# rojas-diego/tokengeex

Measured on AMD Instinct MI355X. Metric: MB/s raw bytes encoded (and tokens/s) at 32K/64K vocab, 1/2/4/8 GPUs, higher is better.
Workload: dtype f64

## Files before the change

### tokengeex_amd/csrc/encode2.hip

```cpp
#include <hip/hip_runtime.h>
#include <stdint.h>

#include "device_common.h"
#include "kernels.h"
#include "trace_body.h"

namespace tgx {

constexpr uint32_t kNoStep2 = 0xFFu;
constexpr uint32_t kRows2Bytes = 64u * 32u * 8u;
constexpr uint64_t kHiHalf = 0xFFFFFFFF00000000ULL;

template <int U>
__device__ __forceinline__ void relax2_step(double sv, double& acc, uint32_t& bpv, uint32_t& fin, uint32_t& fhi) {
    constexpr uint64_t MU = (1ULL << U) | (1ULL << (32 + U));
    fin = sel_u32(MU, bpv, fin);
    fhi = sel_u32(MU, (uint32_t)((uint64_t)__double_as_longlong(acc) >> 32), fhi);
    const double b0 = readlane_f64(acc, (uint32_t)U), b1 = readlane_f64(acc, 32u + (uint32_t)U);
    const double best = sel_f64(kHiHalf, b1, b0);
    const double cand = best + sv;
    const uint64_t take = __builtin_amdgcn_fcmp(cand, acc, 2 ) | MU;
    acc = sel_f64(take, cand, acc);
    bpv = sel_imm_u32<U>(take, bpv);
}
// ... 74 lines not shown
            if (alive) {
                const uint32_t c = (bytes[d >> 2] >> ((d & 3) * 8)) & 0xFFu;
                const uint32_t t = base ^ c;
                const uint4 rec = load_rec(trie, t);
                alive = rec.x == cur;
                if (alive) {
                    cur = t;
                    base = rec.y & 0x7FFFFFFFu;
                    bool term = (rec.y >> 31) != 0u;
                    if (DROPOUT) {
                        if (term && d >= 1) term = P.dropout < dropout_u01(P.seed, s, pg, (uint32_t)d + 1u);
                    }
                    if (term) scw[((uint32_t)d + l) & 31u] = __hiloint2double((int)rec.w, (int)rec.z);
                }
            }
        }
        __builtin_amdgcn_wave_barrier();
        {
            const uint32_t* __restrict__ np = wp + 8;
#pragma unroll
            for (int q = 0; q < 9; ++q) wn[q] = np[q];
        }

        uint32_t fin = kNoStep2, fhi = 0xFFF00000u;
        {
            const double* scr = sc + r * 1024u + ((l - 1u) & 31u);
            double sv[16];
#pragma unroll
            for (int u = 0; u < 16; ++u) sv[u] = scr[u * 32];
            relax2_step<0>(sv[0], acc, bpv, fin, fhi);
            relax2_step<1>(sv[1], acc, bpv, fin, fhi);
            relax2_step<2>(sv[2], acc, bpv, fin, fhi);
            relax2_step<3>(sv[3], acc, bpv, fin, fhi);
            relax2_step<4>(sv[4], acc, bpv, fin, fhi);
            relax2_step<5>(sv[5], acc, bpv, fin, fhi);
            relax2_step<6>(sv[6], acc, bpv, fin, fhi);
            relax2_step<7>(sv[7], acc, bpv, fin, fhi);
            relax2_step<8>(sv[8], acc, bpv, fin, fhi);
            relax2_step<9>(sv[9], acc, bpv, fin, fhi);
            relax2_step<10>(sv[10], acc, bpv, fin, fhi);
            relax2_step<11>(sv[11], acc, bpv, fin, fhi);
            relax2_step<12>(sv[12], acc, bpv, fin, fhi);
            relax2_step<13>(sv[13], acc, bpv, fin, fhi);
            relax2_step<14>(sv[14], acc, bpv, fin, fhi);
            relax2_step<15>(sv[15], acc, bpv, fin, fhi);
#pragma unroll
            for (int u = 0; u < 16; ++u) sv[u] = scr[(u + 16) * 32];
            relax2_step<16>(sv[0], acc, bpv, fin, fhi);
            relax2_step<17>(sv[1], acc, bpv, fin, fhi);
            relax2_step<18>(sv[2], acc, bpv, fin, fhi);
            relax2_step<19>(sv[3], acc, bpv, fin, fhi);
            relax2_step<20>(sv[4], acc, bpv, fin, fhi);
            relax2_step<21>(sv[5], acc, bpv, fin, fhi);
            relax2_step<22>(sv[6], acc, bpv, fin, fhi);
            relax2_step<23>(sv[7], acc, bpv, fin, fhi);
            relax2_step<24>(sv[8], acc, bpv, fin, fhi);
            relax2_step<25>(sv[9], acc, bpv, fin, fhi);
            relax2_step<26>(sv[10], acc, bpv, fin, fhi);
            relax2_step<27>(sv[11], acc, bpv, fin, fhi);
            relax2_step<28>(sv[12], acc, bpv, fin, fhi);
            relax2_step<29>(sv[13], acc, bpv, fin, fhi);
            relax2_step<30>(sv[14], acc, bpv, fin, fhi);
            relax2_step<31>(sv[15], acc, bpv, fin, fhi);
        }
        __builtin_amdgcn_wave_barrier();
        const bool reached = fhi != 0xFFF00000u;

        if (live && pg >= 1u && pg <= n) {
            const uint8_t b = reached ? (uint8_t)((l - fin - 1u) & 31u) : (uint8_t)0xFF;
            __builtin_nontemporal_store(b, P.bp8 + bp8_base(beg, s) + (PERM ? bp8_perm(pg - 1u) : pg - 1u));
        }
        if (live) {
            const uint32_t left = n - p0;
            if (left < 32u) {
                if (left == l) P.status[s] = (n == 0u || reached) ? 1u : 0u;
                need_new = true;
            } else {
                p0 += 32u;
            }
        }
    }
}

template <bool PERM, bool CARRY>
__global__ __launch_bounds__(256) void trace32_kernel(EncodeParams P) {
    __shared__ typename TraceRingEntry<CARRY>::type ring_all[4][kTraceRing];
    trace_body<32, PERM, false, CARRY>(P, ring_all[threadIdx.x >> 6]);
}

hipError_t launch_encode2(const EncodeParams& p, uint32_t num_cus, bool permuted, hipStream_t stream) {
    const uint32_t waves = 5, bpc = 2;
    const uint64_t want = (p.n_samples + 2 * waves - 1) / (2 * waves);
    const uint32_t blocks = (uint32_t)(want < (uint64_t)num_cus * bpc ? (want ? want : 1) : (uint64_t)num_cus * bpc);
    auto fn = p.dropout > 0.0 ? (permuted ? encode2_kernel<true, true> : encode2_kernel<true, false>)
                              : (permuted ? encode2_kernel<false, true> : encode2_kernel<false, false>);
    hipError_t e = hipFuncSetAttribute(reinterpret_cast<const void*>(fn), hipFuncAttributeMaxDynamicSharedMemorySize, 160 * 1024);
    if (e != hipSuccess) return e;
    hipLaunchKernelGGL(fn, dim3(blocks), dim3(64u * waves), waves * kRows2Bytes, stream, p);
    return hipGetLastError();
}
hipError_t launch_trace32(const EncodeParams& p, uint32_t blocks, bool permuted, hipStream_t stream) {
    auto fn = permuted ? (p.trace_carry ? trace32_kernel<true, true> : trace32_kernel<true, false>)
                       : (p.trace_carry ? trace32_kernel<false, true> : trace32_kernel<false, false>);
    hipLaunchKernelGGL(fn, dim3(blocks), dim3(256), 0, stream, p);
    return hipGetLastError();
}

}
```

### tokengeex_amd/csrc/kernels.h

```cpp
#pragma once
#include <hip/hip_runtime.h>
#include <stdint.h>

#include "decode.h"
#include "spans.h"

namespace tgx {

struct EncodeParams {
    const uint8_t* text;
    const uint64_t* offs;
    const uint32_t* order;
    uint64_t n_samples;
    const void* trie;
    const uint32_t* tokid;
    uint32_t root_base;
    uint32_t n_slots;
    uint32_t lm;
    uint32_t* bp;
    uint32_t* tmp;
    uint32_t* counts;
    uint32_t* status;
    uint8_t* bp8;
    const void* tokhash;
    uint32_t tokhash_mask;
    uint32_t tokhash_seed;
    unsigned long long* err_sample;
    unsigned long long* queue;
    unsigned long long* redo_count;
    uint32_t* redo_list;
    double dropout;
    uint64_t seed;
    uint32_t flags;
    unsigned long long* stamps;
    uint32_t trace_carry;
};

struct Encode5Params {
    const void* trie8;
    uint32_t trie_bytes;
    const double* values;
    uint32_t root_base;
    uint32_t n_values;
    uint32_t n_hot;
    uint32_t claim_chunk;
    uint32_t list_off, root_off, idx_off;
    uint32_t ctrl_off, ring_off, ring_slots;
    uint32_t pool;
    unsigned int* started;
};

struct CompactParams {
    const uint64_t* offs;
    const uint32_t* order;
    uint64_t n_samples;
    const uint32_t* tmp;
    const uint64_t* out_offs;
    uint32_t* ids;
};

struct EstepParams {
    const uint8_t* text;
    const uint64_t* offs;
    const uint32_t* order;
    uint64_t n_samples;
    const void* trie_fwd;
    const void* trie_rev;
    uint32_t root_fwd, root_rev;
    uint32_t lm;
    uint64_t snippet_len;
    double* alpha;
    double* expected_slot;
    uint32_t n_slots_rev, n_replicas;
    double* logz_sum;
    unsigned long long* err_sample;
    double dropout;
    uint64_t seed;
};

hipError_t launch_pair_keys(const uint32_t* ids, const uint64_t* out_offs, uint64_t n_samples, uint32_t shift,
                            unsigned long long sentinel, unsigned long long* keys, uint32_t blocks, hipStream_t stream);
hipError_t pair_sort_temp_bytes(uint64_t n, size_t* bytes);
hipError_t pair_sort(void* temp, size_t temp_bytes, const unsigned long long* in, unsigned long long* out,
                     uint64_t n, unsigned int end_bit, hipStream_t stream);
hipError_t pair_rle_temp_bytes(uint64_t n, size_t* bytes);
hipError_t pair_rle(void* temp, size_t temp_bytes, const unsigned long long* sorted, uint64_t n,
                    unsigned long long* unique_out, unsigned int* counts_out, unsigned int* n_runs_out,
                    hipStream_t stream);

hipError_t pair_count_sort_temp_bytes(uint64_t n, size_t* bytes);
hipError_t pair_count_sort(void* temp, size_t temp_bytes, const unsigned int* counts_in, unsigned int* counts_out,
                           const unsigned long long* keys_in, unsigned long long* keys_out, uint64_t n,
                           hipStream_t stream);
hipError_t launch_pair_expand(const unsigned long long* keys, const unsigned int* cnt, uint64_t n, uint32_t shift,
                              unsigned long long* out_keys, unsigned long long* out_counts, hipStream_t stream);
constexpr uint32_t kHistMaxVocab = 36864;
hipError_t launch_ids_histogram(const uint32_t* ids, uint64_t n, uint32_t vocab, unsigned long long* out, uint32_t blocks,
                                hipStream_t stream);
hipError_t ids_sort_temp_bytes(uint64_t n, size_t* bytes);
hipError_t ids_sort(void* temp, size_t temp_bytes, const uint32_t* in, uint32_t* out, uint64_t n,
                    unsigned int end_bit, hipStream_t stream);
hipError_t ids_rle_temp_bytes(uint64_t n, size_t* bytes);
hipError_t ids_rle(void* temp, size_t temp_bytes, const uint32_t* sorted, uint64_t n, uint32_t* unique_out,
                   unsigned int* counts_out, unsigned int* n_runs_out, hipStream_t stream);

struct Estep4Params {
    const uint8_t* text;
    const uint64_t* soffs;
    const uint32_t* order;
    uint64_t n_snips;
    const uint32_t* snip_sample;
    const uint64_t* snip_base;
    const void* trie_fwd;
    const void* trie_rev;
    uint32_t root_fwd, root_rev;
    double* alpha;
    double* zarr;
    int32_t* alpha_exp;
// ... 241 lines not shown
```

### tokengeex_amd/csrc/kernels.hip

```cpp
#include <hip/hip_runtime.h>
#include <stdint.h>

#include <rocprim/device/device_scan.hpp>
#include <rocprim/iterator/transform_iterator.hpp>

#include "kernels.h"
#include "trace_body.h"
#include "device_common.h"

namespace tgx {

struct WaveCtx {
    const uint4* __restrict__ trie;
    uint32_t root_base;
    double dropout;
    uint64_t seed;
    bool use_dropout;
    uint32_t flags;
};

__device__ __forceinline__ void block_generic(const WaveCtx& C, const uint8_t* __restrict__ text, uint32_t n,
                                              uint32_t s, uint32_t p0, uint32_t lane, uint32_t LM,
                                              double* sc, uint32_t* hl, uint8_t* txt, uint32_t* __restrict__ bp,
                                              double& acc, uint32_t& bpv, uint64_t& reach, uint32_t& reach_n) {
// ... 394 lines not shown
                    }
                }
            }
        }
        __builtin_amdgcn_wave_barrier();
        TGX_STAMP(2)
        {
            const uint32_t* __restrict__ np = wp + 4 * PPL;
#pragma unroll
            for (int q = 0; q <= 4 * PPL; ++q) wn[q] = np[q];
        }

        uint32_t fin[PPL];
        bool reached[PPL];
#pragma unroll
        for (int g = 0; g < PPL; ++g) {
            fin[g] = kNoStep;
            reached[g] = false;
            if (P.flags & 2u) continue;
            const double* scr = reinterpret_cast<const double*>(wbase + g * kRows4GroupBytes) + r * 256u + ((l - 1u) & 15u);
            double sv[16];
#pragma unroll
            for (int u = 0; u < 16; ++u) sv[u] = scr[u * 16];
            uint32_t fhi = 0xFFF00000u;
            relax5_step<0>(sv[0], acc, bpv, fin[g], fhi);
            relax5_step<1>(sv[1], acc, bpv, fin[g], fhi);
            relax5_step<2>(sv[2], acc, bpv, fin[g], fhi);
            relax5_step<3>(sv[3], acc, bpv, fin[g], fhi);
            relax5_step<4>(sv[4], acc, bpv, fin[g], fhi);
            relax5_step<5>(sv[5], acc, bpv, fin[g], fhi);
            relax5_step<6>(sv[6], acc, bpv, fin[g], fhi);
            relax5_step<7>(sv[7], acc, bpv, fin[g], fhi);
            relax5_step<8>(sv[8], acc, bpv, fin[g], fhi);
            relax5_step<9>(sv[9], acc, bpv, fin[g], fhi);
            relax5_step<10>(sv[10], acc, bpv, fin[g], fhi);
            relax5_step<11>(sv[11], acc, bpv, fin[g], fhi);
            relax5_step<12>(sv[12], acc, bpv, fin[g], fhi);
            relax5_step<13>(sv[13], acc, bpv, fin[g], fhi);
            relax5_step<14>(sv[14], acc, bpv, fin[g], fhi);
            relax5_step<15>(sv[15], acc, bpv, fin[g], fhi);
            reached[g] = fhi != 0xFFF00000u;
        }
        __builtin_amdgcn_wave_barrier();
        TGX_STAMP(3)

        uint8_t* const bpw = P.bp8 + bp8_base(beg, s);
#pragma unroll
        for (int g = 0; g < PPL; ++g)
            if (live && pg[g] >= 1u && pg[g] <= n) {
                const uint32_t b = reached[g] ? ((l - fin[g] - 1u) & 15u) : 0xFFu;
                const uint32_t j = pg[g] - 1u, kq = (j >> 4) & 3u;
                pk = (kq == 0u) ? b : (pk | (b << (8u * kq)));
                pk_j = j;
                pk_dirty = true;
                if (kq == 3u) {
                    __builtin_nontemporal_store(pk, reinterpret_cast<uint32_t*>(bpw + (bp8_perm(j) & ~3u)));
                    pk_dirty = false;
                }
            }
        if (live && n - p0 < SPAN && pk_dirty) {
            __builtin_nontemporal_store(pk, reinterpret_cast<uint32_t*>(bpw + (bp8_perm(pk_j) & ~3u)));
            pk_dirty = false;
        }
        if (live) {
            const uint32_t left = n - p0;
            if (left < SPAN) {
#pragma unroll
                for (int g = 0; g < PPL; ++g)
                    if (left == 16u * g + l) P.status[s] = (n == 0u || reached[g]) ? 1u : 0u;
                need_new = true;
            } else {
                p0 += SPAN;
            }
        }
        TGX_STAMP(4)
    }
    if (STAMP && lane == 0 && P.stamps) {
        unsigned long long* o = P.stamps + (size_t)(blockIdx.x * wpb + wave) * 8u;
        for (int i = 0; i < 5; ++i) o[i] = seg[i];
        o[5] = iters;
    }
}

template <bool STAMP, bool CARRY>
__global__ __launch_bounds__(256) void trace_kernel(EncodeParams P) {
    __shared__ typename TraceRingEntry<CARRY>::type ring_all[4][kTraceRing];
    trace_body<16, true, STAMP, CARRY>(P, ring_all[threadIdx.x >> 6]);
}

__global__ __launch_bounds__(1024) void scan_counts_kernel(const uint32_t* __restrict__ counts,
                                                           uint64_t* __restrict__ offsets,
                                                           uint64_t n) {
    __shared__ uint64_t wsum[16];
    __shared__ uint64_t carry_s;
    constexpr uint32_t E = 8;
    const uint32_t tid = threadIdx.x, lane = tid & 63u, wave = tid >> 6;
    if (tid == 0) carry_s = 0;
    __syncthreads();
    for (uint64_t base = 0; base < n; base += 1024u * E) {
        const uint64_t i0 = base + (uint64_t)tid * E;
        uint32_t c[E];
        uint64_t v = 0;
#pragma unroll
        for (uint32_t e = 0; e < E; ++e) {
            c[e] = (i0 + e < n) ? counts[i0 + e] : 0u;
            v += c[e];
        }
        uint64_t x = v;
        for (int off = 1; off < 64; off <<= 1) {
            uint64_t y = __shfl_up(x, off);
            if ((int)lane >= off) x += y;
        }
        if (lane == 63) wsum[wave] = x;
        __syncthreads();
        uint64_t wprefix = 0;
        for (uint32_t w = 0; w < wave; ++w) wprefix += wsum[w];
        const uint64_t carry = carry_s;
        uint64_t run = carry + wprefix + x - v;
#pragma unroll
        for (uint32_t e = 0; e < E; ++e) {
            if (i0 + e < n) offsets[i0 + e] = run;
            run += c[e];
        }
        __syncthreads();
        if (tid == 1023) carry_s = run;
        __syncthreads();
    }
    if (tid == 0) offsets[n] = carry_s;
}

template <bool ROWS>
__global__ __launch_bounds__(256) void compact_kernel(CompactParams P) {
    const uint32_t lane = threadIdx.x & 63u;
    const uint32_t sub = ROWS ? (lane & 15u) : lane, width = ROWS ? 16u : 64u;
    const uint64_t n_units = (uint64_t)gridDim.x * 4u * (ROWS ? 4u : 1u);
    const uint32_t wave_id = blockIdx.x * 4u + (threadIdx.x >> 6);
    for (uint64_t k = ROWS ? (uint64_t)wave_id * 4u + (lane >> 4) : (uint64_t)wave_id; k < P.n_samples; k += n_units) {
        const uint32_t s = ROWS ? (uint32_t)k : P.order[k];
        const uint64_t end = P.offs[s + 1];
        const uint64_t o0 = P.out_offs[s];
        const uint32_t cnt = (uint32_t)(P.out_offs[s + 1] - o0);
        const uint32_t* __restrict__ src = P.tmp + (end - cnt);
        uint32_t* __restrict__ dst = P.ids + o0;
        struct __attribute__((packed, aligned(4))) Ids4 { uint32_t w[4]; };
        const uint32_t body = cnt & ~3u;
        for (uint32_t i = sub * 4u; i < body; i += width * 4u)
            *reinterpret_cast<Ids4*>(dst + i) = *reinterpret_cast<const Ids4*>(src + i);
        if (body + sub < cnt) dst[body + sub] = src[body + sub];
    }
}


static int lmt_for(uint32_t lm) { return lm <= 16u ? 16 : (lm <= 32u ? 32 : 0); }
uint32_t encode_effective_lm(uint32_t lm) {
    const int t = lmt_for(lm);
    return t ? (uint32_t)t : lm;
}

uint32_t encode_waves_per_block(uint32_t lm) {
    uint32_t w = (64u * 1024u) / wave_lds_bytes(encode_effective_lm(lm));
    return w < 1u ? 1u : (w > 4u ? 4u : w);
}
uint32_t encode_lds_bytes_per_block(uint32_t lm) {
    return encode_waves_per_block(lm) * wave_lds_bytes(encode_effective_lm(lm));
}

typedef void (*encode_fn)(EncodeParams);
static encode_fn pick_kernel(uint32_t lm) {
    const int t = lmt_for(lm);
    if (t == 16) return encode_kernel<16>;
    if (t == 32) return encode_kernel<32>;
    return encode_kernel<0>;
}

hipError_t launch_encode(const EncodeParams& p, uint32_t blocks, hipStream_t stream) {
    const uint32_t lds = encode_lds_bytes_per_block(p.lm);
    const dim3 block(64u * encode_waves_per_block(p.lm));
    hipLaunchKernelGGL(pick_kernel(p.lm), dim3(blocks), block, lds, stream, p);
    return hipGetLastError();
}

hipError_t encode_max_blocks_per_cu(uint32_t lm, int* out) {
    const uint32_t lds = encode_lds_bytes_per_block(lm);
    const int threads = (int)(64u * encode_waves_per_block(lm));
    if (lds > 160u * 1024u) return hipErrorInvalidValue;
    encode_fn fn = pick_kernel(lm);
    hipError_t e = hipFuncSetAttribute(reinterpret_cast<const void*>(fn),
                                       hipFuncAttributeMaxDynamicSharedMemorySize, (int)lds);
    if (e != hipSuccess) return e;
    return hipOccupancyMaxActiveBlocksPerMultiprocessor(out, fn, threads, lds);
}

typedef void (*encode4_fn)(EncodeParams);
static encode4_fn pick_encode4(bool dropout, int ppl, bool stamp, bool root) {
    if (stamp) return encode4_kernel<false, 1, true, false>;
    if (root) return dropout ? encode4_kernel<true, 1, false, true> : encode4_kernel<false, 1, false, true>;
    if (ppl == 1) return dropout ? encode4_kernel<true, 1, false, false> : encode4_kernel<false, 1, false, false>;
    if (ppl == 2) return dropout ? encode4_kernel<true, 2, false, false> : encode4_kernel<false, 2, false, false>;
    return dropout ? encode4_kernel<true, 4, false, false> : encode4_kernel<false, 4, false, false>;
}
uint32_t encode4_group_bytes() { return kRows4GroupBytes; }
uint32_t encode4_lds_bytes(int waves, int ppl, bool root) {
    return (root ? 4096u : 0u) + (uint32_t)waves * (uint32_t)ppl * kRows4GroupBytes;
}
hipError_t encode4_waves_per_simd(bool dropout, int ppl, bool root, int* out) {
    root = root && ppl == 1;
    hipFuncAttributes attr;
    hipError_t e = hipFuncGetAttributes(&attr, reinterpret_cast<const void*>(pick_encode4(dropout, ppl, false, root)));
    if (e != hipSuccess) return e;
    const int regs = (attr.numRegs + 7) & ~7;
    *out = regs > 0 ? (512 / regs > 8 ? 8 : 512 / regs) : 8;
    return hipSuccess;
}
hipError_t launch_encode4(const EncodeParams& p, int ppl, int waves, uint32_t blocks, bool root, hipStream_t stream) {
    const bool stamp = p.stamps != nullptr;
    root = root && !stamp && ppl == 1;
    encode4_fn fn = pick_encode4(p.dropout > 0.0, ppl, stamp, root);
    hipError_t e = hipFuncSetAttribute(reinterpret_cast<const void*>(fn), hipFuncAttributeMaxDynamicSharedMemorySize, 160 * 1024);
    if (e != hipSuccess) return e;
    hipLaunchKernelGGL(fn, dim3(blocks), dim3(64u * (uint32_t)waves), encode4_lds_bytes(waves, stamp ? 1 : ppl, root), stream, p);
    return hipGetLastError();
}
hipError_t launch_trace(const EncodeParams& p, uint32_t blocks, hipStream_t stream) {
    if (p.stamps)
        hipLaunchKernelGGL((trace_kernel<true, false>), dim3(blocks), dim3(256), 0, stream, p);
    else if (p.trace_carry)
        hipLaunchKernelGGL((trace_kernel<false, true>), dim3(blocks), dim3(256), 0, stream, p);
    else
        hipLaunchKernelGGL((trace_kernel<false, false>), dim3(blocks), dim3(256), 0, stream, p);
    return hipGetLastError();
}

struct WidenU32 {
    __host__ __device__ uint64_t operator()(uint32_t x) const { return (uint64_t)x; }
};
hipError_t scan_temp_bytes(uint64_t n, size_t* bytes) {
    *bytes = 0;
    if (n <= 65536) return hipSuccess;
    auto in = rocprim::make_transform_iterator((const uint32_t*)nullptr, WidenU32());
    return rocprim::exclusive_scan(nullptr, *bytes, in, (uint64_t*)nullptr, (uint64_t)0, (size_t)(n + 1), rocprim::plus<uint64_t>());
}
hipError_t launch_scan(uint32_t* counts, uint64_t* offsets, uint64_t n, void* temp, size_t temp_bytes, hipStream_t stream) {
    if (n <= 65536 || !temp) {
        hipLaunchKernelGGL(scan_counts_kernel, dim3(1), dim3(1024), 0, stream, counts, offsets, n);
        return hipGetLastError();
    }
    hipError_t e = hipMemsetAsync(counts + n, 0, 4, stream);
    if (e != hipSuccess) return e;
    auto in = rocprim::make_transform_iterator((const uint32_t*)counts, WidenU32());
    return rocprim::exclusive_scan(temp, temp_bytes, in, offsets, (uint64_t)0, (size_t)(n + 1), rocprim::plus<uint64_t>(), stream);
}

hipError_t launch_compact(const CompactParams& p, uint32_t blocks, bool rows, hipStream_t stream) {
    if (rows)
        hipLaunchKernelGGL(compact_kernel<true>, dim3(blocks), dim3(256), 0, stream, p);
    else
        hipLaunchKernelGGL(compact_kernel<false>, dim3(blocks), dim3(256), 0, stream, p);
    return hipGetLastError();
}

}
```

### tokengeex_amd/csrc/tgx_api.cpp

```cpp
#include <hip/hip_runtime.h>

#include <algorithm>
#include <unordered_set>
#include <cstdarg>
#include <cstddef>
#include <cstdio>
#include <cstdlib>
#include <cmath>
#include <cstring>
#include <chrono>
#include <condition_variable>
#include <memory>
#include <mutex>
#include <new>
#include <numeric>
#include <string>
#include <thread>
#include <vector>

#include "../../include/tgx.h"
#include "api_internal.h"
#include "assemble.h"
#include "decode.h"
#include "kernels.h"
// ... 473 lines not shown

tgx_status ensure_value_ranks(tgx_model* m, const tgx_corpus* c) {
    if (m->values_ranked || !m->have_trie8 || !c->n_bytes) return TGX_OK;
    m->values_ranked = true;
    const char* vr = knob("TGX_VALUE_RANK");
    if (vr && strcmp(vr, "model") == 0) return TGX_OK;
    if (m->n_values <= tgx::encode5_max_hot(false, 13, 3, 160u * 1024u) && !(vr && strcmp(vr, "counts") == 0)) return TGX_OK;
    tgx::HostPhases hp("ensure_value_ranks");
    HIP_TRY(hipSetDevice(m->device));
    const uint32_t nv = m->n_values, chunk = 65536u;
    const uint64_t stride = std::max<uint64_t>(chunk, (c->n_bytes + 63) / 64);
    const size_t cb = ((size_t)nv + 1) * 4 + 256;
    Pass pass(m);
    unsigned int* d_cnt = nullptr;
    uint32_t* d_perm = nullptr;
    if (pass.alloc(cb, &d_cnt) != hipSuccess || pass.alloc(cb, &d_perm) != hipSuccess)
        return fail(TGX_ERR_DEVICE, "out of device memory (value counts)");
    std::vector<unsigned int> cnt((size_t)nv + 1, 0u);
    std::vector<double> values((size_t)nv + 1), wvalues;
    bool ok = hipMemsetAsync(d_cnt, 0, cb, m->stream) == hipSuccess &&
              tgx::launch_value_count(c->d_text, c->n_bytes, chunk, stride, m->d_trie8, (uint32_t)m->flat.table.size(), m->root_base8, nv,
                                      std::max<uint32_t>(1, m->flat.max_token_len), d_cnt, (uint32_t)m->num_cus, m->stream) == hipSuccess &&
              hipMemcpyAsync(cnt.data(), d_cnt, ((size_t)nv + 1) * 4, hipMemcpyDeviceToHost, m->stream) == hipSuccess &&
              hipMemcpyAsync(values.data(), m->d_values, ((size_t)nv + 1) * 8, hipMemcpyDeviceToHost, m->stream) == hipSuccess;
    if (ok && m->have_wvalues) {
        wvalues.resize((size_t)nv + 1);
        ok = hipMemcpyAsync(wvalues.data(), m->d_wvalues, ((size_t)nv + 1) * 8, hipMemcpyDeviceToHost, m->stream) == hipSuccess;
    }
    if (!ok || hipStreamSynchronize(m->stream) != hipSuccess)
        return fail(TGX_ERR_DEVICE, "value count pass failed: %s", hipGetErrorString(hipGetLastError()));
    hp.mark("value counts");
    std::vector<uint32_t> order(nv);
    for (uint32_t r = 0; r < nv; r++) order[r] = r + 1u;
    std::stable_sort(order.begin(), order.end(), [&](uint32_t a, uint32_t b) { return cnt[a] > cnt[b]; });
    std::vector<uint32_t> perm((size_t)nv + 1, 0u);
    std::vector<double> v2((size_t)nv + 1), w2(wvalues.size());
    v2[0] = values[0];
    if (!w2.empty()) w2[0] = wvalues[0];
    unsigned long long total = 0, run = 0;
    for (uint32_t r = 0; r < nv; r++) total += cnt[order[r]];
    std::vector<double> cov((size_t)nv + 1, 0.0);
    for (uint32_t r = 0; r < nv; r++) {
        perm[order[r]] = r + 1u;
        v2[r + 1u] = values[order[r]];
        if (!w2.empty()) w2[r + 1u] = wvalues[order[r]];
        run += cnt[order[r]];
        cov[r + 1u] = total ? (double)run / (double)total : 1.0;
    }
    cov[nv] = 1.0;
    ok = hipMemcpyAsync(d_perm, perm.data(), ((size_t)nv + 1) * 4, hipMemcpyHostToDevice, m->stream) == hipSuccess &&
         tgx::launch_rank_remap(m->d_trie8, (uint32_t)m->flat.table.size(), d_perm, m->stream) == hipSuccess &&
         hipMemcpyAsync(m->d_values, v2.data(), ((size_t)nv + 1) * 8, hipMemcpyHostToDevice, m->stream) == hipSuccess &&
         (w2.empty() || hipMemcpyAsync(m->d_wvalues, w2.data(), ((size_t)nv + 1) * 8, hipMemcpyHostToDevice, m->stream) == hipSuccess) &&
         hipStreamSynchronize(m->stream) == hipSuccess;
    if (!ok) return fail(TGX_ERR_DEVICE, "value re-rank failed: %s", hipGetErrorString(hipGetLastError()));
    m->value_coverage = std::move(cov);
    hp.mark("re-rank");
    return pass.done();
}

tgx::EncodeParams base_encode_params(const tgx_model* m, const tgx_corpus* c, uint64_t seed) {
    tgx::EncodeParams p{};
    p.text = c->d_text;
    p.offs = c->d_offs;
    p.order = c->d_order;
    p.n_samples = c->n_samples;
    p.trie = m->d_trie;
    p.tokid = m->d_tokid;
    p.root_base = m->flat.table[0].base & ~tgx::kTerminalBit;
    p.lm = m->lm;
    p.n_slots = (uint32_t)m->flat.table.size();
    p.bp = c->d_bp;
    p.tmp = c->d_tmp;
    p.counts = c->d_counts;
    p.status = c->d_status;
    p.bp8 = reinterpret_cast<uint8_t*>(c->d_bp.get());
    p.tokhash = m->d_tokhash;
    p.tokhash_mask = m->tokhash.mask;
    p.tokhash_seed = m->tokhash.seed;
    p.err_sample = &m->d_ctrl->err;
    p.queue = &m->d_ctrl->queue;
    p.seed = seed;
    p.trace_carry = (c->n_samples && c->n_bytes / c->n_samples < 2048) ? 1u : 0u;
    return p;
}

tgx_status redo_long_matches(tgx_model* m, tgx_corpus* c, const tgx::EncodeParams& p) {
    unsigned long long n_redo = 0;
    HIP_TRY(hipMemcpyAsync(&n_redo, &m->d_ctrl->encode_redo, 8, hipMemcpyDeviceToHost, m->stream));
    HIP_TRY(hipStreamSynchronize(m->stream));
    if (n_redo > c->n_samples) return fail(TGX_ERR_DEVICE, "redo list longer than the batch");
    m->last_redo_samples = n_redo;
    if (n_redo) {
        tgx::EncodeParams q = p;
        q.order = c->d_counts;
        q.n_samples = n_redo;
        HIP_TRY(hipMemsetAsync(&m->d_ctrl->queue, 0x00, 8, m->stream));
        time_begin(m, "encode2_kernel");
        HIP_TRY(tgx::launch_encode2(q, (uint32_t)m->num_cus, true, m->stream));
        time_end(m);
    }
    return TGX_OK;
}

tgx_status run_encode_kernel(tgx_model* m, tgx_corpus* c, double dropout, uint64_t seed, Pass& pass) {
    tgx_status st = ensure_scratch(c);
    if (st != TGX_OK) return st;
    HIP_TRY(hipMemsetAsync(&m->d_ctrl->queue, 0x00, 8, m->stream));
    HIP_TRY(hipMemsetAsync(&m->d_ctrl->err, 0xFF, 8, m->stream));
    tgx::EncodeParams p = base_encode_params(m, c, seed);
    p.dropout = dropout;
    if (const char* e = knob("TGX_TRACE_CARRY")) p.trace_carry = atoi(e) ? 1u : 0u;
    p.flags = debug_flags();
    const char* force = knob("TGX_PATH");
    const bool use4 = m->lm <= 16 && m->scores_finite && m->d_tokhash && !(force && strcmp(force, "fused") == 0);
    const bool use2 = !use4 && m->lm <= 32 && m->scores_finite && m->d_tokhash && !(force && strcmp(force, "fused") == 0);
    const bool long_tokens = m->lm > 16;
    const bool use5 = (use4 || use2) && m->have_trie8 &&
                      !(force && (strcmp(force, "rows4") == 0 || strcmp(force, "rows2") == 0 || strcmp(force, "rows4l") == 0));
    if (debug_on())
        fprintf(stderr, "[tgx] encode: S=%llu N=%llu lm=%u path=%s slots=%zu root_base=%u values=%u\n",
                (unsigned long long)c->n_samples, (unsigned long long)c->n_bytes, p.lm, use4 ? (use5 ? "rows5" : "rows4") : (use2 ? "rows2" : "fused"),
                m->flat.table.size(), p.root_base, m->n_values);
    if (use5) {
        {
            const tgx_status rst = ensure_value_ranks(m, c);
            if (rst != TGX_OK) return rst;
        }
        m->last_redo_samples = 0;
        int e6_bpc = 2;
        if (const char* e = knob("TGX_E6_BPC")) e6_bpc = std::min(4, std::max(1, atoi(e)));
        uint32_t n_hot6 = std::min(m->n_values, tgx::encode6_max_hot(160u * 1024u / (uint32_t)e6_bpc, 0u));
        uint32_t pool6 = 0;
        bool e6_usable = true;
        if (n_hot6 < m->n_values) {
            pool6 = 128;
            if (const char* e = knob("TGX_E6_POOL")) pool6 = (uint32_t)std::min(192, std::max(0, atoi(e)));
            if ((uint64_t)m->n_values + tgx::encode6_pool_total(pool6) > 65535ull) {
                pool6 = 0;
                e6_usable = knob("TGX_E6_POOL") != nullptr || knob("TGX_LONG_THRESHOLD") != nullptr;
            }
            n_hot6 = std::min(m->n_values, tgx::encode6_max_hot(160u * 1024u / (uint32_t)e6_bpc, pool6));
        }
        n_hot6 = knob_cap_hot("TGX_E5_HOT", n_hot6);
        const bool cold6 = n_hot6 < m->n_values;
        uint64_t n_long = 0;
        uint32_t corun_cus = 0;
        if (c->n_samples && !long_tokens && e6_usable) {
            const auto count_ge = [&](uint64_t thr) {
                return (uint64_t)(std::partition_point(c->h_sorted_len.begin(), c->h_sorted_len.end(),
                                                       [thr](uint32_t len) { return len >= thr; }) - c->h_sorted_len.begin());
            };
            if (const char* e = knob("TGX_LONG_THRESHOLD")) {
                const uint64_t thr = (uint64_t)std::max(0ll, atoll(e));
                if (thr) n_long = count_ge(thr);
            } else {
                const double N = (double)c->n_bytes;
                const double c5 = m->n_values > tgx::encode5_max_hot(false, 8, 4, 160u * 1024u) ? 0.135e-6 : 0.108e-6;
                auto cost = [&](uint64_t k) {
                    const double bytes_long = k ? (double)c->h_sorted_cum[k - 1] : 0.0;
                    const double t6 = k ? std::max((double)c->h_sorted_len[0] * (cold6 ? 0.042e-6 : 0.0369e-6), bytes_long / (cold6 ? 46e9 : 55e9)) + 20e-6 : 0.0;
                    const double rest_max = k < c->n_samples ? (double)c->h_sorted_len[k] : 0.0;
                    const double t5 = std::max(rest_max * c5, (N - bytes_long) / 88e9);
                    return t6 + t5;
                };
                double best = cost(0);
                for (uint64_t thr = 1024; thr <= c->max_len; thr *= 2) {
                    const uint64_t k = count_ge(thr);
                    const double ck = cost(k);
                    if (k && ck < best * 0.9) {
                        best = ck;
                        n_long = k;
                    }
                }
                const double c6 = cold6 ? 0.042e-6 : 0.0369e-6, r6 = (cold6 ? 46e9 : 55e9) / (double)m->num_cus;
                double best_co = best * 0.9;
                uint64_t k_co = 0;
                static const uint64_t thrs[] = {8192, 12288, 16384, 24576, 32768, 40960, 49152};
                static const uint32_t shares[] = {32, 48, 64, 96, 128, 160, 192};
                const bool corun_off = (knob("TGX_CORUN") && atoi(knob("TGX_CORUN")) == 0) || m->corun_wait_timeouts != 0 ||
                                       m->n_values > tgx::encode5_max_hot(false, 8, 4, 160u * 1024u);
                for (uint64_t thr : thrs) {
                    if (corun_off || thr > c->max_len || e6_bpc != 2) break;
                    const uint64_t k = count_ge(thr);
                    if (!k || k >= c->n_samples) continue;
                    const double bytes_long = (double)c->h_sorted_cum[k - 1];
                    const double r_max = (double)c->h_sorted_len[k], r_bytes = N - bytes_long;
                    for (uint32_t X : shares) {
                        if ((int)X >= m->num_cus) break;
                        const double t6 = std::max((double)c->h_sorted_len[0] * c6, bytes_long / (X * r6)) + 20e-6;
                        const double t5 = std::max(r_max * 0.12e-6, r_bytes / ((double)(m->num_cus - (int)X) / (double)m->num_cus * 70e9));
                        const double t = std::max(t5, t6);
                        if (t < best_co) {
                            best_co = t;
                            k_co = k;
// ... 87 lines not shown
        if (const char* e = knob("TGX_CLAIM_CHUNK")) q.claim_chunk = (uint32_t)std::min(64, std::max(1, atoi(e)));
        m->last_long_samples = n_long;
        m->last_corun_cus = n_long ? corun_cus : 0u;
        tgx::EncodeParams p6 = p;
        tgx::Encode5Params q6 = q;
        uint32_t blocks6 = 0;
        if (n_long) {
            p6.n_samples = n_long;
            blocks6 = (uint32_t)std::min<uint64_t>((n_long + 3) / 4, (uint64_t)(corun_cus ? (int)corun_cus : m->num_cus) * (uint64_t)e6_bpc);
            q6.n_hot = n_hot6;
            q6.pool = cold6 ? pool6 : 0u;
            if (!corun_cus) {
                time_begin(m, "encode6_kernel");
                HIP_TRY(tgx::launch_encode6(p6, q6, cold6, blocks6, m->stream));
                time_end(m);
                HIP_TRY(hipMemsetAsync(&m->d_ctrl->queue, 0x00, 8, m->stream));
            } else {
                if (!m->stream2) {
                    HIP_TRY(hipStreamCreateWithFlags(&m->stream2, hipStreamNonBlocking));
                    HIP_TRY(hipEventCreateWithFlags(&m->ev_fork, hipEventDisableTiming));
                    HIP_TRY(hipEventCreateWithFlags(&m->ev_join, hipEventDisableTiming));
                    HIP_TRY(hipHostMalloc((void**)&m->h_started, 64, hipHostMallocMapped | hipHostMallocPortable));
                }
                *reinterpret_cast<volatile unsigned int*>(m->h_started) = 0u;
                q.started = m->h_started;
                p6.queue = &m->d_ctrl->queue6;
                HIP_TRY(hipMemsetAsync(&m->d_ctrl->queue6, 0x00, 8, m->stream));
                HIP_TRY(hipEventRecord(m->ev_fork, m->stream));
                HIP_TRY(hipStreamWaitEvent(m->stream2, m->ev_fork, 0));
            }
            p.order = c->d_order + n_long;
            p.n_samples = c->n_samples - n_long;
        }
        const Stamps stamps5 = stamps_begin(m, pass, '1', (size_t)blocks5 * (size_t)waves);
        p.stamps = stamps5.d;
        time_begin(m, "encode5_kernel");
        {
            if (long_tokens) {
                p.redo_count = &m->d_ctrl->encode_redo;
                p.redo_list = c->d_counts;
                HIP_TRY(hipMemsetAsync(&m->d_ctrl->encode_redo, 0x00, 8, m->stream));
            }
            const hipError_t le = tgx::launch_encode5(p, q, cold, ppl, long_tokens, compact, waves, blocks5, corun_cus && n_long ? 84u * 1024u : 0u, m->stream);
            if (le != hipSuccess) return fail(TGX_ERR_DEVICE, "encode5 launch failed: %s", hipGetErrorString(le));
        }
        bool joined = false, joined_slot = false;
        if (n_long && corun_cus) {
            const bool slot = m->n_timed + 1 < kMaxTimed;
            if (slot) {
                KernelTime& tb = m->timed[m->n_timed + 1];
                tb.name = "encode6_kernel";
                tb.used = true;
                (void)hipEventRecord(tb.start, m->stream2);
            }
            {
                const auto t0 = std::chrono::steady_clock::now();
                volatile unsigned int* started = m->h_started;
                bool timed_out = false;
                while (*started < blocks5 && !(timed_out = std::chrono::steady_clock::now() - t0 >= std::chrono::milliseconds(2))) {
                }
                if (timed_out && *started < blocks5) m->corun_wait_timeouts++;
            }
            const hipError_t l6 = tgx::launch_encode6(p6, q6, cold6, blocks6, m->stream2);
            if (slot) (void)hipEventRecord(m->timed[m->n_timed + 1].stop, m->stream2);
            (void)hipEventRecord(m->ev_join, m->stream2);
            if (l6 != hipSuccess) return fail(TGX_ERR_DEVICE, "encode6 launch failed: %s", hipGetErrorString(l6));
            joined = true;
            joined_slot = slot;
        }
        time_end(m);
        if (joined) {
            if (joined_slot) m->n_timed++;
            HIP_TRY(hipStreamWaitEvent(m->stream, m->ev_join, 0));
        }
        if (stamps5.d) stamps_report(m, stamps5, ppl, "encode5 stamps", "iteration", {"switch", "text+reset", "walk", "relax", "store"});
        p.stamps = nullptr;
        if (long_tokens) {
            const tgx_status rst = redo_long_matches(m, c, p);
            if (rst != TGX_OK) return rst;
        }
        p.order = c->d_order;
        p.n_samples = c->n_samples;
        const uint32_t blocks_t = trace_blocks(m, c->n_samples);
        time_begin(m, long_tokens ? "trace32_kernel" : "trace_kernel");
        if (long_tokens) HIP_TRY(tgx::launch_trace32(p, blocks_t, true, m->stream));
        else HIP_TRY(tgx::launch_trace(p, blocks_t, m->stream));
        time_end(m);
    } else if (use4) {
        int ppl = 1, waves = 10, bpc = 2;
        const double gbps4[3] = {60.0, 50.0, 34.0}, chain4_ms[3] = {13.5, 10.7, 9.1};
        auto cost4 = [&](double bytes, double longest, int* ppl_out) {
            double best_t = 0;
            int best_ppl = 1;
            for (int i = 0; i < 3; i++) {
                const double t = std::max(bytes / (gbps4[i] * 1e9), longest / 65536.0 * chain4_ms[i] * 1e-3);
                if (i == 0 || t < best_t * 0.95) {
                    best_t = t;
                    best_ppl = 1 << i;
                }
            }
            if (ppl_out) *ppl_out = best_ppl;
            return best_t;
        };
        m->last_long_samples = 0;
        m->last_redo_samples = 0;
        cost4((double)c->n_bytes, c->n_samples ? (double)c->h_sorted_len[0] : 0.0, &ppl);
        if (const char* e = knob("TGX_PPL")) {
            const int v = atoi(e);
            if (v == 1 || v == 2 || v == 4) ppl = v;
        }
        if (ppl == 2) { waves = 5; bpc = 2; }
        if (ppl == 4) { waves = 5; bpc = 1; }
        knob_int("TGX_WAVES", 1, 16, &waves);
        knob_int("TGX_BPC", 1, 8, &bpc);
        bool root = ppl == 1;
        if (const char* e = knob("TGX_ROOT")) root = root && atoi(e) != 0;
        while (waves > 1 && tgx::encode4_lds_bytes(waves, ppl, root) > (160u * 1024u) / (uint32_t)bpc) waves--;
        {
            int per_simd = 0;
            HIP_TRY(tgx::encode4_waves_per_simd(dropout > 0.0, ppl, root, &per_simd));
            if (bpc * ((waves + 3) / 4) > per_simd && ppl == 1) {
                waves = 4;
                bpc = std::min(5, per_simd);
                root = false;
                HIP_TRY(tgx::encode4_waves_per_simd(dropout > 0.0, ppl, root, &per_simd));
            }
            m->last_encode_waves_per_cu = std::min(bpc * ((waves + 3) / 4), per_simd) * 4 >= bpc * waves
                                              ? bpc * waves
                                              : per_simd / ((waves + 3) / 4) * waves;
        }
        const uint64_t rows_per_block = 4 * (uint64_t)waves;
        const uint32_t blocks4 = (uint32_t)std::max<uint64_t>(
            1, std::min<uint64_t>((p.n_samples + rows_per_block - 1) / rows_per_block, (uint64_t)m->num_cus * bpc));
        Stamps stamps4;
        if (dropout <= 0.0 && ppl == 1) stamps4 = stamps_begin(m, pass, '1', (size_t)blocks4 * (size_t)waves);
        p.stamps = stamps4.d;
        time_begin(m, "encode4_kernel");
        HIP_TRY(tgx::launch_encode4(p, ppl, waves, blocks4, root, m->stream));
        time_end(m);
        if (stamps4.d) stamps_report(m, stamps4, 0, "stamps", "iteration", {"switch", "text", "walk", "relax", "store"});
        p.stamps = nullptr;
        p.order = c->d_order;
        p.n_samples = c->n_samples;
        time_begin(m, "trace_kernel");
        HIP_TRY(tgx::launch_trace(p, trace_blocks(m, c->n_samples), m->stream));
        time_end(m);
    } else if (use2) {
        const bool rows2 = force && strcmp(force, "rows2") == 0;
        m->last_redo_samples = 0;
        if (!rows2) {
            p.redo_count = &m->d_ctrl->encode_redo;
            p.redo_list = c->d_counts;
            HIP_TRY(hipMemsetAsync(&m->d_ctrl->encode_redo, 0x00, 8, m->stream));
            time_begin(m, "encode4l_kernel");
            HIP_TRY(tgx::launch_encode4l(p, (uint32_t)m->num_cus, m->stream));
            time_end(m);
            const tgx_status rst = redo_long_matches(m, c, p);
            if (rst != TGX_OK) return rst;
        } else {
            time_begin(m, "encode2_kernel");
            HIP_TRY(tgx::launch_encode2(p, (uint32_t)m->num_cus, false, m->stream));
            time_end(m);
        }
        time_begin(m, "trace32_kernel");
        HIP_TRY(tgx::launch_trace32(p, trace_blocks(m, c->n_samples), !rows2, m->stream));
        time_end(m);
    } else {
        time_begin(m, "encode_kernel");
        HIP_TRY(tgx::launch_encode(p, grid_blocks(m, c->n_samples), m->stream));
        time_end(m);
// ... 2866 lines not shown
```

### tokengeex_amd/csrc/trace_body.h

```cpp
#pragma once
#include <hip/hip_runtime.h>
#include <stdint.h>

#include "device_common.h"
#include "kernels.h"

namespace tgx {

constexpr uint32_t kTraceRing = 128;

#define TGX_TRACE_STAMP(i)                                             \
    if (STAMP) {                                                       \
        __builtin_amdgcn_sched_barrier(0);                             \
        const uint64_t _now = (uint64_t)__builtin_amdgcn_s_memtime(); \
        __builtin_amdgcn_s_waitcnt(0xC07F);                            \
        __builtin_amdgcn_sched_barrier(0);                             \
        seg[i] += _now - t_last;                                       \
        t_last = _now;                                                 \
    }

template <bool CARRY> struct TraceRingEntry { using type = uint2; };
template <> struct TraceRingEntry<true> { using type = uint4; };
template <uint32_t LM, bool PERM, bool STAMP, bool CARRY>
__device__ __forceinline__ void trace_body(const EncodeParams& P, typename TraceRingEntry<CARRY>::type* ring) {
    static_assert(LM == 16 || LM == 32, "token lengths of up to 16 or 32 bytes");
    constexpr uint32_t LMASK = LM - 1u;
    constexpr int NW = (int)LM / 4;
    const uint32_t lane = threadIdx.x & 63u;
    const uint32_t wpb = blockDim.x >> 6;
    const uint32_t n_waves = gridDim.x * wpb;
    const uint32_t wave_id = (uint32_t)__builtin_amdgcn_readfirstlane((int)(blockIdx.x * wpb + (threadIdx.x >> 6)));
    const uint4* __restrict__ table = reinterpret_cast<const uint4*>(P.tokhash);
    uint64_t seg[6] = {0, 0, 0, 0, 0, 0};
    uint64_t t_last = STAMP ? (uint64_t)__builtin_amdgcn_s_memtime() : 0;
    uint32_t iters = 0;
    const uint64_t n_rounds = (P.n_samples + n_waves - 1) / n_waves;
    constexpr uint32_t kNone = 0xFFFFFFFFu;
    auto sample_of_round = [&](uint64_t rnd) -> uint32_t {
        const uint64_t k = rnd * n_waves + ((rnd & 1u) ? (uint64_t)(n_waves - 1u - wave_id) : (uint64_t)wave_id);
        return (rnd < n_rounds && k < P.n_samples) ? P.order[k] : kNone;
    };
    struct MetaRaw {
        uint64_t beg, end;
        uint32_t reach;
    };
    struct Meta {
        uint32_t s;
        uint64_t beg;
        uint32_t n, reach_n;
    };
    auto meta_request = [&](uint32_t smp) -> MetaRaw {
        MetaRaw r{0, 0, 1u};
        if (smp != kNone) {
            r.beg = P.offs[smp];
            r.end = P.offs[smp + 1];
            r.reach = P.status[smp];
        }
        return r;
    };
    auto meta_read = [&](uint32_t smp, const MetaRaw& r) -> Meta {
        Meta mt{smp, 0, 0, 1u};
        if (smp != kNone) {
            mt.beg = first_u64(r.beg);
            mt.n = (uint32_t)(first_u64(r.end) - mt.beg);
            mt.reach_n = (mt.n == 0) ? 1u : (uint32_t)__builtin_amdgcn_readfirstlane((int)r.reach);
        }
        return mt;
    };
    auto first_window = [&](const Meta& mt) -> uint32_t {
        if (mt.s == kNone || mt.n == 0 || !mt.reach_n || (P.flags & 4u)) return 0u;
        const uint8_t* __restrict__ bpn = P.bp8 + bp8_base(mt.beg, mt.s);
        const uint32_t wq0 = (mt.n - 1u) & ~63u;
        return (wq0 + lane < mt.n) ? (uint32_t)bpn[PERM ? bp8_perm(wq0 + lane) : wq0 + lane] : 0u;
    };
    uint32_t head = 0, fill = 0;
    uint64_t flush_beg = 0, flush_out_top = 0;
    auto lookup = [&](uint32_t m) {
        if (lane < m && !(P.flags & 16u)) {
            const auto e = ring[(head + lane) & (kTraceRing - 1u)];
            uint32_t len;
            uint64_t end, out;
            if constexpr (CARRY) {
                len = e.y >> 16;
                end = ((uint64_t)(e.y & 0xFFFFu) << 32) | e.x;
                out = ((uint64_t)e.w << 32) | e.z;
            } else {
                len = e.y;
                end = flush_beg + e.x;
                out = flush_out_top - 1u - lane;
            }
            struct __attribute__((packed, aligned(1))) Bytes16 { uint32_t w[4]; };
            const Bytes16* __restrict__ src = reinterpret_cast<const Bytes16*>(P.text + (end - len));
            uint32_t b[8] = {0, 0, 0, 0, 0, 0, 0, 0};
#pragma unroll
            for (int j = 0; j < NW; j += 4) {
                const Bytes16 raw = src[j / 4];
#pragma unroll
                for (int i = 0; i < 4; ++i) {
                    const uint32_t nb = len > 4u * (j + i) ? len - 4u * (j + i) : 0u;
                    b[j + i] = nb >= 4u ? raw.w[i] : (raw.w[i] & ((1u << (8u * nb)) - 1u));
                }
            }
            const uint64_t hk = LM == 16 ? tok_hash64_dev(b[0], b[1], b[2], b[3], len, P.tokhash_seed)
                                         : tok_hash64_long_dev(b, len, P.tokhash_seed);
            uint32_t slot = (uint32_t)hk & P.tokhash_mask;
            uint32_t id = 0;
            bool found = false;
            for (uint32_t probe = 0; probe <= P.tokhash_mask && !found; ++probe) {
                const uint4 t = load_rec(table, slot);
                if (t.w == 0u) break;
                if (t.x == (uint32_t)hk && t.y == (uint32_t)(hk >> 32)) {
                    id = t.z;
                    found = true;
                }
                slot = (slot + 1u) & P.tokhash_mask;
            }
            if (!found) atomicMin(P.err_sample, (unsigned long long)((end - len) & ((1ULL << 62) - 1ULL)) | (1ULL << 62));
            P.tmp[out] = id;
        }
        if constexpr (!CARRY) flush_out_top -= m;
        head = (head + m) & (kTraceRing - 1u);
        fill -= m;
    };
    Meta cur;
    {
        const uint32_t s0 = (uint32_t)__builtin_amdgcn_readfirstlane((int)sample_of_round(0));
        cur = meta_read(s0, meta_request(s0));
    }
    uint32_t s_next_raw = sample_of_round(1);
    uint32_t h_first = first_window(cur);
    for (uint64_t rnd = 0; rnd < n_rounds; ++rnd) {
        const uint32_t s_next = (uint32_t)__builtin_amdgcn_readfirstlane((int)s_next_raw);
        const uint32_t s_after_raw = sample_of_round(rnd + 2);
        const MetaRaw nxt_raw = meta_request(s_next);
        const uint32_t s = cur.s;
        const uint64_t beg = cur.beg;
        const uint32_t n = cur.n;
        const uint32_t reach_n = cur.reach_n;
        const bool have = s != kNone;
        const uint8_t* __restrict__ bp = P.bp8 + (have ? bp8_base(beg, s) : 0);
        uint32_t total = 0;
        uint64_t out_top = beg + n;
        flush_beg = beg;
        flush_out_top = out_top;
        int64_t q = (have && reach_n) ? (int64_t)n - 1 : (int64_t)-1;
        if (P.flags & 4u) q = -1;

        uint32_t h_cur = h_first;
        TGX_TRACE_STAMP(0)
        while (q >= 0) {
            iters++;
            const uint32_t wq = (uint32_t)q & ~63u;
            const uint32_t idx = wq + lane;
            const uint32_t h = h_cur;
            uint32_t prev = lane - ((h & LMASK) + 1u);
            asm volatile("" : "+v"(prev) : : "memory");
            uint32_t h_next = 0;
            if (wq >= 64u) h_next = (uint32_t)bp[PERM ? bp8_perm(wq - 64u + lane) : wq - 64u + lane];
            TGX_TRACE_STAMP(1)
            uint64_t ends = 0;
            int32_t qq = (int32_t)((uint32_t)q - wq);
            while (qq >= 0) {
                asm("s_bitset1_b64 %0, %1" : "+s"(ends) : "s"(qq));
                qq = (int32_t)readlane_u32(prev, (uint32_t)qq);
            }
            q = (int64_t)wq + qq;
            const uint32_t cnt = (uint32_t)__popcll(ends);
            TGX_TRACE_STAMP(2)
            if ((ends >> lane) & 1ULL) {
                const uint32_t below = __builtin_amdgcn_mbcnt_hi((uint32_t)(ends >> 32), __builtin_amdgcn_mbcnt_lo((uint32_t)ends, 0u));
                if constexpr (CARRY) {
                    const uint64_t end = beg + idx + 1u, out = out_top - 1u - (cnt - 1u - below);
                    ring[(head + fill + (cnt - 1u - below)) & (kTraceRing - 1u)] =
                        make_uint4((uint32_t)end, (uint32_t)(end >> 32) | (((h & LMASK) + 1u) << 16), (uint32_t)out, (uint32_t)(out >> 32));
                } else {
                    ring[(head + fill + (cnt - 1u - below)) & (kTraceRing - 1u)] = make_uint2(idx + 1u, (h & LMASK) + 1u);
                }
            }
            fill += cnt;
            total += cnt;
            out_top -= cnt;
            __builtin_amdgcn_wave_barrier();
            if (fill >= 64u) lookup(64u);
            TGX_TRACE_STAMP(3)
            h_cur = h_next;
        }
        const Meta nxt = meta_read(s_next, nxt_raw);
        h_first = first_window(nxt);
        if constexpr (!CARRY) {
            if (fill) lookup(fill);
        }
        if (have && lane == 0) {
            P.counts[s] = total;
            if (!reach_n) atomicMin(P.err_sample, (unsigned long long)s);
        }
        cur = nxt;
        s_next_raw = s_after_raw;
    }
    if (fill) lookup(fill);
    if (STAMP && lane == 0 && P.stamps) {
        unsigned long long* o = P.stamps + (size_t)wave_id * 8u;
        for (int i = 0; i < 5; ++i) o[i] = seg[i];
        o[5] = iters;
    }
}

}
```

Measured before the change: 68950.

## Use pointer-jumping strides in trace backtrack to cut serial readlane hops

```diff
diff --git a/tokengeex_amd/csrc/encode2.hip b/tokengeex_amd/csrc/encode2.hip
--- a/tokengeex_amd/csrc/encode2.hip
+++ b/tokengeex_amd/csrc/encode2.hip
@@ -180,10 +180,10 @@
     }
 }
 
-template <bool PERM, bool CARRY>
+template <bool PERM, bool CARRY, int K>
 __global__ __launch_bounds__(256) void trace32_kernel(EncodeParams P) {
     __shared__ typename TraceRingEntry<CARRY>::type ring_all[4][kTraceRing];
-    trace_body<32, PERM, false, CARRY>(P, ring_all[threadIdx.x >> 6]);
+    trace_body<32, PERM, false, CARRY, K>(P, ring_all[threadIdx.x >> 6]);
 }
 
 hipError_t launch_encode2(const EncodeParams& p, uint32_t num_cus, bool permuted, hipStream_t stream) {
@@ -197,10 +197,23 @@
     hipLaunchKernelGGL(fn, dim3(blocks), dim3(64u * waves), waves * kRows2Bytes, stream, p);
     return hipGetLastError();
 }
+template <bool PERM, bool CARRY>
+static void launch_trace32_stride(const EncodeParams& p, uint32_t blocks, hipStream_t stream) {
+    switch (p.trace_stride) {
+        case 1: hipLaunchKernelGGL((trace32_kernel<PERM, CARRY, 1>), dim3(blocks), dim3(256), 0, stream, p); break;
+        case 2: hipLaunchKernelGGL((trace32_kernel<PERM, CARRY, 2>), dim3(blocks), dim3(256), 0, stream, p); break;
+        case 3: hipLaunchKernelGGL((trace32_kernel<PERM, CARRY, 3>), dim3(blocks), dim3(256), 0, stream, p); break;
+        default: hipLaunchKernelGGL((trace32_kernel<PERM, CARRY, 0>), dim3(blocks), dim3(256), 0, stream, p); break;
+    }
+}
 hipError_t launch_trace32(const EncodeParams& p, uint32_t blocks, bool permuted, hipStream_t stream) {
-    auto fn = permuted ? (p.trace_carry ? trace32_kernel<true, true> : trace32_kernel<true, false>)
-                       : (p.trace_carry ? trace32_kernel<false, true> : trace32_kernel<false, false>);
-    hipLaunchKernelGGL(fn, dim3(blocks), dim3(256), 0, stream, p);
+    if (permuted) {
+        if (p.trace_carry) launch_trace32_stride<true, true>(p, blocks, stream);
+        else launch_trace32_stride<true, false>(p, blocks, stream);
+    } else {
+        if (p.trace_carry) launch_trace32_stride<false, true>(p, blocks, stream);
+        else launch_trace32_stride<false, false>(p, blocks, stream);
+    }
     return hipGetLastError();
 }
 
diff --git a/tokengeex_amd/csrc/kernels.h b/tokengeex_amd/csrc/kernels.h
--- a/tokengeex_amd/csrc/kernels.h
+++ b/tokengeex_amd/csrc/kernels.h
@@ -6,6 +6,8 @@
 #include "spans.h"
 
 namespace tgx {
+
+constexpr uint32_t kTraceStride = 2;
 
 struct EncodeParams {
     const uint8_t* text;
@@ -34,6 +36,7 @@
     uint32_t flags;
     unsigned long long* stamps;
     uint32_t trace_carry;
+    uint32_t trace_stride;
 };
 
 struct Encode5Params {
diff --git a/tokengeex_amd/csrc/kernels.hip b/tokengeex_amd/csrc/kernels.hip
--- a/tokengeex_amd/csrc/kernels.hip
+++ b/tokengeex_amd/csrc/kernels.hip
@@ -500,10 +500,10 @@
     }
 }
 
-template <bool STAMP, bool CARRY>
+template <bool STAMP, bool CARRY, int K>
 __global__ __launch_bounds__(256) void trace_kernel(EncodeParams P) {
     __shared__ typename TraceRingEntry<CARRY>::type ring_all[4][kTraceRing];
-    trace_body<16, true, STAMP, CARRY>(P, ring_all[threadIdx.x >> 6]);
+    trace_body<16, true, STAMP, CARRY, K>(P, ring_all[threadIdx.x >> 6]);
 }
 
 __global__ __launch_bounds__(1024) void scan_counts_kernel(const uint32_t* __restrict__ counts,
@@ -639,13 +639,22 @@
     hipLaunchKernelGGL(fn, dim3(blocks), dim3(64u * (uint32_t)waves), encode4_lds_bytes(waves, stamp ? 1 : ppl, root), stream, p);
     return hipGetLastError();
 }
+template <bool STAMP, bool CARRY>
+static void launch_trace_stride(const EncodeParams& p, uint32_t blocks, hipStream_t stream) {
+    switch (p.trace_stride) {
+        case 1: hipLaunchKernelGGL((trace_kernel<STAMP, CARRY, 1>), dim3(blocks), dim3(256), 0, stream, p); break;
+        case 2: hipLaunchKernelGGL((trace_kernel<STAMP, CARRY, 2>), dim3(blocks), dim3(256), 0, stream, p); break;
+        case 3: hipLaunchKernelGGL((trace_kernel<STAMP, CARRY, 3>), dim3(blocks), dim3(256), 0, stream, p); break;
+        default: hipLaunchKernelGGL((trace_kernel<STAMP, CARRY, 0>), dim3(blocks), dim3(256), 0, stream, p); break;
+    }
+}
 hipError_t launch_trace(const EncodeParams& p, uint32_t blocks, hipStream_t stream) {
     if (p.stamps)
-        hipLaunchKernelGGL((trace_kernel<true, false>), dim3(blocks), dim3(256), 0, stream, p);
+        launch_trace_stride<true, false>(p, blocks, stream);
     else if (p.trace_carry)
-        hipLaunchKernelGGL((trace_kernel<false, true>), dim3(blocks), dim3(256), 0, stream, p);
+        launch_trace_stride<false, true>(p, blocks, stream);
     else
-        hipLaunchKernelGGL((trace_kernel<false, false>), dim3(blocks), dim3(256), 0, stream, p);
+        launch_trace_stride<false, false>(p, blocks, stream);
     return hipGetLastError();
 }
 
diff --git a/tokengeex_amd/csrc/tgx_api.cpp b/tokengeex_amd/csrc/tgx_api.cpp
--- a/tokengeex_amd/csrc/tgx_api.cpp
+++ b/tokengeex_amd/csrc/tgx_api.cpp
@@ -579,6 +579,7 @@
     p.queue = &m->d_ctrl->queue;
     p.seed = seed;
     p.trace_carry = (c->n_samples && c->n_bytes / c->n_samples < 2048) ? 1u : 0u;
+    p.trace_stride = tgx::kTraceStride;
     return p;
 }
 
@@ -608,6 +609,7 @@
     tgx::EncodeParams p = base_encode_params(m, c, seed);
     p.dropout = dropout;
     if (const char* e = knob("TGX_TRACE_CARRY")) p.trace_carry = atoi(e) ? 1u : 0u;
+    if (const char* e = knob("TGX_TRACE_STRIDE")) p.trace_stride = (uint32_t)std::min(3, std::max(0, atoi(e)));
     p.flags = debug_flags();
     const char* force = knob("TGX_PATH");
     const bool use4 = m->lm <= 16 && m->scores_finite && m->d_tokhash && !(force && strcmp(force, "fused") == 0);
@@ -861,10 +863,15 @@
         p.order = c->d_order;
         p.n_samples = c->n_samples;
         const uint32_t blocks_t = trace_blocks(m, c->n_samples);
+        Stamps stamps_t;
+        if (!long_tokens) stamps_t = stamps_begin(m, pass, '2', (size_t)blocks_t * 4);
+        p.stamps = stamps_t.d;
         time_begin(m, long_tokens ? "trace32_kernel" : "trace_kernel");
         if (long_tokens) HIP_TRY(tgx::launch_trace32(p, blocks_t, true, m->stream));
         else HIP_TRY(tgx::launch_trace(p, blocks_t, m->stream));
         time_end(m);
+        if (stamps_t.d) stamps_report(m, stamps_t, 0, "trace stamps", "window", {"setup", "loads", "hops", "append+lookups", "-"});
+        p.stamps = nullptr;
     } else if (use4) {
         int ppl = 1, waves = 10, bpc = 2;
         const double gbps4[3] = {60.0, 50.0, 34.0}, chain4_ms[3] = {13.5, 10.7, 9.1};
diff --git a/tokengeex_amd/csrc/trace_body.h b/tokengeex_amd/csrc/trace_body.h
--- a/tokengeex_amd/csrc/trace_body.h
+++ b/tokengeex_amd/csrc/trace_body.h
@@ -19,9 +19,47 @@
         t_last = _now;                                                 \
     }
 
+__device__ __forceinline__ int32_t trace_lane_addr(int32_t p) {
+    return (p < 0 ? 0 : p) << 2;
+}
+__device__ __forceinline__ int32_t trace_square(int32_t p) {
+    const int32_t got = __builtin_amdgcn_ds_bpermute(trace_lane_addr(p), p);
+    return p < 0 ? p : got;
+}
+template <int K>
+__device__ __forceinline__ uint64_t trace_hops(uint32_t prev, int32_t& qq) {
+    static_assert(K >= 0 && K <= 3, "strides of 1, 2, 4, 8 tokens");
+    if constexpr (K == 0) {
+        uint64_t ends = 0;
+        while (qq >= 0) {
+            asm("s_bitset1_b64 %0, %1" : "+s"(ends) : "s"(qq));
+            qq = (int32_t)readlane_u32(prev, (uint32_t)qq);
+        }
+        return ends;
+    } else {
+        int32_t p[K + 1];
+        p[0] = (int32_t)prev;
+#pragma unroll
+        for (int k = 1; k <= K; ++k) p[k] = trace_square(p[k - 1]);
+        uint64_t visited = 0;
+        while (qq >= 0) {
+            asm("s_bitset1_b64 %0, %1" : "+s"(visited) : "s"(qq));
+            qq = (int32_t)readlane_u32((uint32_t)p[K], (uint32_t)qq);
+        }
+        uint64_t on = visited;
+#pragma unroll
+        for (int k = K - 1; k >= 0; --k) {
+            const bool send = __builtin_amdgcn_inverse_ballot_w64(on) && p[k] >= 0;
+            const int32_t got = __builtin_amdgcn_ds_permute(send ? trace_lane_addr(p[k]) : 63 << 2, 1);
+            on |= __builtin_amdgcn_ballot_w64(got != 0) & ~(1ULL << 63);
+        }
+        return on;
+    }
+}
+
 template <bool CARRY> struct TraceRingEntry { using type = uint2; };
 template <> struct TraceRingEntry<true> { using type = uint4; };
-template <uint32_t LM, bool PERM, bool STAMP, bool CARRY>
+template <uint32_t LM, bool PERM, bool STAMP, bool CARRY, int K>
 __device__ __forceinline__ void trace_body(const EncodeParams& P, typename TraceRingEntry<CARRY>::type* ring) {
     static_assert(LM == 16 || LM == 32, "token lengths of up to 16 or 32 bytes");
     constexpr uint32_t LMASK = LM - 1u;
@@ -158,12 +196,8 @@
             uint32_t h_next = 0;
             if (wq >= 64u) h_next = (uint32_t)bp[PERM ? bp8_perm(wq - 64u + lane) : wq - 64u + lane];
             TGX_TRACE_STAMP(1)
-            uint64_t ends = 0;
             int32_t qq = (int32_t)((uint32_t)q - wq);
-            while (qq >= 0) {
-                asm("s_bitset1_b64 %0, %1" : "+s"(ends) : "s"(qq));
-                qq = (int32_t)readlane_u32(prev, (uint32_t)qq);
-            }
+            const uint64_t ends = trace_hops<K>(prev, qq);
             q = (int64_t)wq + qq;
             const uint32_t cnt = (uint32_t)__popcll(ends);
             TGX_TRACE_STAMP(2)
```

After: 70960 (median of 6 runs). 1.03x the previous value.
